# ATTron/astroz

Measured on AMD Instinct MI355X. Metric: propagations/sec, 13,478 sats x 1,440 times, at 1/2/4/8 MI355X, higher is better.
Workload: dtype f64

## Files before the change

astroz_amd/_native.py:

```python
import ctypes as C
import os

import numpy as np

_HERE = os.path.dirname(os.path.abspath(__file__))
LIB_PATH = os.environ.get("ASTROZ_AMD_LIB") or os.path.join(_HERE, "libastroz_hip.so")

WGS84, WGS72 = 0, 1
OUT_TEME, OUT_ECEF, OUT_GEODETIC, OUT_TOPOCENTRIC = 0, 1, 2, 3
SAT_MAJOR, TIME_MAJOR = 0, 1
OUTPUT_MODES = {"teme": OUT_TEME, "ecef": OUT_ECEF, "geodetic": OUT_GEODETIC, "topocentric": OUT_TOPOCENTRIC}
PASS_DTYPE = np.dtype([("t_rise_min", "<f8"), ("t_culm_min", "<f8"), ("t_set_min", "<f8"), ("max_elevation_rad", "<f8"),
                       ("rise_azimuth_rad", "<f8"), ("set_azimuth_rad", "<f8"), ("flags", "<u4"), ("grid_rise", "<u4"),
                       ("grid_culm", "<u4"), ("grid_set", "<u4")])
PASS_UP_AT_START, PASS_UP_AT_END, PASS_CUT_BY_ERROR = 1, 2, 4
ECLIPSE_DTYPE = np.dtype([("t_entry_min", "<f8"), ("t_exit_min", "<f8"), ("flags", "<u4"), ("grid_entry", "<u4"),
                          ("grid_exit", "<u4"), ("reserved", "<u4")])
ECLIPSE_IN_AT_START, ECLIPSE_IN_AT_END, ECLIPSE_CUT_BY_ERROR = 1, 2, 4
SHADOW_UMBRA, SHADOW_PENUMBRA = 0, 1
SHADOW_KINDS = {"umbra": SHADOW_UMBRA, "penumbra": SHADOW_PENUMBRA}
ACCESS_DTYPE = np.dtype([("t_start_min", "<f8"), ("t_end_min", "<f8"), ("min_range_km", "<f8"), ("flags", "<u4"),
                         ("grid_start", "<u4"), ("grid_end", "<u4"), ("grid_min_range", "<u4")])
ACCESS_OPEN_AT_START, ACCESS_OPEN_AT_END, ACCESS_CUT_BY_ERROR = 1, 2, 4
CONJUNCTION_DTYPE = np.dtype([("t_tca_min", "<f8"), ("miss_km", "<f8"), ("rel_speed_km_s", "<f8"), ("target", "<u4"),
                              ("sat", "<u4"), ("grid_index", "<u4"), ("reserved", "<u4")])

COVERAGE_DTYPE = np.dtype([("mean_in_view", "<f8"), ("max_gap_min", "<f8"), ("n_covered", "<u4"), ("min_in_view", "<u4"),
                           ("max_in_view", "<u4"), ("n_gaps", "<u4"), ("grid_gap_start", "<u4"), ("grid_gap_end", "<u4"),
                           ("flags", "<u4"), ("reserved", "<u4")])
COVERAGE_GAP_AT_START, COVERAGE_GAP_AT_END = 1, 2

AZ_ERR_HIP = -200
PATH_ROWS_FAST, PATH_TILES_FAST, PATH_ROWS_GENERIC, PATH_LANE_SAT, PATH_DEEP_ROWS, PATH_QUASI_UNIFORM, PATH_COLS_FAST, PATH_HOST_STEP = 1, 2, 4, 8, 16, 32, 64, 128

EXPORTS = [
    "astroz_version", "astroz_init", "astroz_deinit", "tle_parse", "tle_free",
    "tle_get_satellite_number", "tle_get_epoch", "tle_get_inclination", "tle_get_eccentricity",
    "tle_get_mean_motion", "sgp4_init", "sgp4_free", "sgp4_propagate", "sgp4_propagate_batch",
    "azh_device_count", "azh_last_error", "azh_parse_tle_lines", "azh_constellation_from_tle_text",
    "azh_constellation_from_tle_lines", "azh_constellation_from_elements", "azh_constellation_subset", "azh_constellation_free",
    "azh_num_satellites", "azh_num_sgp4", "azh_num_sdp4", "azh_get_epochs", "azh_get_status",
    "azh_get_field", "azh_propagate_host", "azh_propagate_device", "azh_propagate_device_cached", "azh_propagate_device_window",
    "azh_propagate_jd_host", "azh_synchronize", "azh_propagate_one_host", "azh_set_time_tile", "azh_set_timing", "azh_set_fast_path", "azh_set_tile_kernel", "azh_set_graphs", "azh_set_f32_arithmetic", "azh_set_f32_mode",
    "azh_last_kernel_ms", "azh_last_path", "azh_last_one_stats", "azh_last_window_tiers", "azh_set_host_copy_threads", "azh_set_host_points", "azh_get_host_points", "azh_selftest_coords", "azh_selftest_host_step", "azh_host_alloc", "azh_host_free", "azh_host_pool_stats", "azh_host_pool_trim", "azh_propagate_device_f32", "azh_propagate_device_cached_f32",
    "azh_screen_target_host", "azh_screen_target_device", "azh_coarse_screen_device", "azh_coarse_screen_host",
    "azh_screen_all_host", "azh_constellation_from_omm_json", "azh_propagate_one_device", "azh_selftest_math",
    "azh_parse_tle_text", "azh_parse_omm_json", "azh_set_parse_threads", "coords_julian_to_gmst",
    "azh_group_create_from_tle_text", "azh_group_create_from_omm_json", "azh_group_free", "azh_group_num_satellites",
    "azh_group_num_devices", "azh_group_padded_rows", "azh_group_get_epochs", "azh_group_propagate_host",
    "azh_group_propagate_allgather", "azh_group_screen_target_host", "azh_group_screen_target_device", "azh_group_shard_size",
    "azh_group_shard_rows", "azh_group_synchronize", "azh_screen_track_device", "coords_eci_to_ecef", "coords_ecef_to_geodetic",
    "orbital_hohmann", "orbital_velocity", "orbital_period", "orbital_escape_velocity",
    "azh_coords_topocentric", "azh_set_observer", "azh_find_passes_host", "azh_find_passes_device",
    "azh_find_passes_stations_host", "azh_find_passes_stations_device",
    "azh_coverage_host", "azh_coverage_device",
    "azh_sun_position_teme", "azh_selftest_sun", "azh_shadow_state", "azh_find_eclipses_host", "azh_find_eclipses_device",
    "azh_line_of_sight", "azh_find_access_host", "azh_find_access_device", "azh_find_access_track_device",
    "azh_closest_approach", "azh_find_conjunctions_host", "azh_find_conjunctions_device",
]


def _stations(stations, min_elevation_deg):
    st = np.ascontiguousarray(stations, dtype=np.float64).reshape(-1, 3)
    mk = np.ascontiguousarray(np.broadcast_to(np.asarray(min_elevation_deg, dtype=np.float64), (len(st),)))
    return st, mk


def _targets(targets):
    a = np.atleast_1d(np.asarray(targets))
    if a.ndim != 1 or a.size == 0 or a.dtype == np.bool_ or not np.issubdtype(a.dtype, np.integer) or (a < 0).any():
        raise ValueError("targets must be a satellite index or a non-empty sequence of them")
    return np.ascontiguousarray(a, dtype=np.uintp)


def _min_satellites(k):
    if isinstance(k, bool) or not isinstance(k, (int, np.integer)) or not 1 <= int(k) <= 0xFFFFFFFF:
        raise ValueError("min_satellites must be an integer >= 1")
# ... 143 lines not shown
    L.azh_set_timing.restype = i32
    L.azh_set_fast_path.argtypes = [vp, i32]
    L.azh_set_fast_path.restype = i32
    L.azh_set_tile_kernel.argtypes = [vp, i32]
    L.azh_set_tile_kernel.restype = i32
    L.azh_set_graphs.argtypes = [vp, i32]
    L.azh_set_graphs.restype = i32
    L.azh_set_f32_arithmetic.argtypes = [vp, i32]
    L.azh_set_f32_arithmetic.restype = i32
    L.azh_set_f32_mode.argtypes = [vp, i32]
    L.azh_set_f32_mode.restype = i32
    L.azh_last_kernel_ms.argtypes = [vp]
    L.azh_last_kernel_ms.restype = dbl
    L.azh_set_host_copy_threads.argtypes = [i32]
    L.azh_set_host_copy_threads.restype = None
    L.azh_set_host_points.argtypes = [sz]
    L.azh_set_host_points.restype = None
    L.azh_get_host_points.argtypes = []
    L.azh_get_host_points.restype = sz
    L.azh_host_alloc.argtypes = [C.c_size_t, C.POINTER(C.c_void_p)]
    L.azh_host_alloc.restype = i32
    L.azh_host_free.argtypes = [C.c_void_p]
    L.azh_host_free.restype = None
    L.azh_host_pool_stats.argtypes = [C.POINTER(C.c_size_t), C.POINTER(C.c_size_t)]
    L.azh_host_pool_stats.restype = None
    L.azh_host_pool_trim.argtypes = []
    L.azh_host_pool_trim.restype = None
    L.azh_last_path.argtypes = [vp]
    L.azh_last_path.restype = u32
    L.azh_last_one_stats.argtypes = [vp, vp, vp]
    L.azh_last_one_stats.restype = C.c_int32
    L.azh_last_window_tiers.argtypes = [vp, vp]
    L.azh_last_window_tiers.restype = C.c_int32
    L.azh_propagate_device_f32.argtypes = L.azh_propagate_device.argtypes
    L.azh_propagate_device_f32.restype = i32
    L.azh_propagate_device_cached_f32.argtypes = L.azh_propagate_device_cached.argtypes
    L.azh_propagate_device_cached_f32.restype = i32
    L.azh_screen_target_host.argtypes = [vp, vp, sz, vp, sz, dbl, dbl, vp, vp]
    L.azh_screen_target_host.restype = i32
    L.azh_screen_target_device.argtypes = [vp, vp, sz, vp, sz, dbl, dbl, vp, vp, vp]
    L.azh_screen_target_device.restype = i32
    L.azh_screen_track_device.argtypes = [vp, vp, sz, vp, vp, sz, dbl, vp, vp, vp]
    L.azh_screen_track_device.restype = i32
    L.azh_coarse_screen_device.argtypes = [vp, sz, sz, i32, sz, dbl, vp, vp, vp, sz, C.POINTER(sz), vp]
    L.azh_coarse_screen_device.restype = i32
    L.azh_coarse_screen_host.argtypes = [vp, sz, sz, i32, sz, dbl, vp, vp, vp, sz, C.POINTER(sz), i32]
    L.azh_coarse_screen_host.restype = i32
    L.azh_screen_all_host.argtypes = [vp, vp, sz, vp, dbl, vp, vp, sz, C.POINTER(sz)]
    L.azh_screen_all_host.restype = i32
    L.azh_coords_topocentric.argtypes = [vp, vp, dbl, vp, vp, vp]
    L.azh_coords_topocentric.restype = None
    L.azh_set_observer.argtypes = [vp, dbl, dbl, dbl]
    L.azh_set_observer.restype = i32
    L.azh_find_passes_host.argtypes = [vp, vp, sz, vp, dbl, dbl, vp, sz, vp]
    L.azh_find_passes_host.restype = i32
    L.azh_find_passes_device.argtypes = [vp, vp, sz, vp, dbl, dbl, vp, sz, vp, vp]
    L.azh_find_passes_device.restype = i32
    L.azh_find_passes_stations_host.argtypes = [vp, vp, sz, vp, dbl, vp, vp, sz, vp, sz, vp]
    L.azh_find_passes_stations_host.restype = i32
    L.azh_find_passes_stations_device.argtypes = [vp, vp, sz, vp, dbl, vp, vp, sz, vp, sz, vp, vp]
    L.azh_find_passes_stations_device.restype = i32
    L.azh_coverage_host.argtypes = [vp, vp, sz, vp, dbl, vp, vp, sz, u32, vp, vp]
    L.azh_coverage_host.restype = i32
    L.azh_coverage_device.argtypes = [vp, vp, sz, vp, dbl, vp, vp, sz, u32, vp, vp, vp]
    L.azh_coverage_device.restype = i32
    L.azh_sun_position_teme.argtypes = [dbl, vp]
# ... 381 lines not shown

    def set_fast_path(self, enabled):
        check(lib().azh_set_fast_path(self._h, 1 if enabled else 0), "azh_set_fast_path")

    def set_tile_kernel(self, enabled):
        check(lib().azh_set_tile_kernel(self._h, int(enabled) if not isinstance(enabled, bool) else (1 if enabled else 0)), "azh_set_tile_kernel")

    def set_graphs(self, enabled):
        check(lib().azh_set_graphs(self._h, 1 if enabled else 0), "azh_set_graphs")

    def set_timing(self, enabled):
        check(lib().azh_set_timing(self._h, 1 if enabled else 0), "azh_set_timing")

    def synchronize(self):
        check(lib().azh_synchronize(self._h), "azh_synchronize")

    def last_kernel_ms(self):
        return lib().azh_last_kernel_ms(self._h)

    def last_path(self):
        return int(lib().azh_last_path(self._h))

    def last_one_stats(self):
        a, b = C.c_uint32(0), C.c_uint32(0)
        check(lib().azh_last_one_stats(self._h, C.byref(a), C.byref(b)), "azh_last_one_stats")
        return int(a.value), int(b.value)


    def last_window_tiers(self):
        cnt = (C.c_uint32 * 4)()
        check(lib().azh_last_window_tiers(self._h, cnt), "azh_last_window_tiers")
        return dict(zip(("general", "eps", "ecc", "rejected"), (int(x) for x in cnt)))


class DeviceGroup:

    def __init__(self, text, devices, grav=WGS72, n_chunks=4):
        b = text.encode() if isinstance(text, str) else bytes(text)
        dv = (C.c_int32 * len(devices))(*devices)
        h = C.c_void_p()
        fn = lib().azh_group_create_from_omm_json if b.lstrip()[:1] in (b"{", b"[") else lib().azh_group_create_from_tle_text
        check(fn(b, len(b), grav, dv, len(devices), n_chunks, C.byref(h)), "azh_group_create")
        self._h = h
        self.n = lib().azh_group_num_satellites(h)
        self.n_devices = lib().azh_group_num_devices(h)
        self.padded_rows = lib().azh_group_padded_rows(h)
        self.epochs = np.empty(self.n)
        check(lib().azh_group_get_epochs(h, self.epochs.ctypes.data), "azh_group_get_epochs")

    def close(self):
        if getattr(self, "_h", None):
            lib().azh_group_free(self._h)
            self._h = None

    def __del__(self):
        try:
            self.close()
        except Exception:
            pass

    def _offsets(self, offsets_min):
        if offsets_min is None:
            return None
        off = _f64(offsets_min)
        if off.ndim != 1 or len(off) < self.n:
            raise ValueError("epoch_offsets must have at least num_satellites elements")
# ... 271 lines not shown
```

astroz_amd/csrc/astroz_hip.hip:

```cpp
#include "../../include/astroz_hip.h"

#include <hip/hip_runtime.h>
#include <dlfcn.h>
#include <rccl/rccl.h>

#include <algorithm>
#include <atomic>
#include <cmath>
#include <condition_variable>
#include <deque>
#include <map>
#include <cstdio>
#include <cstdlib>
#include <cstring>
#include <mutex>
#include <new>
#include <memory>
#include <string>
#include <thread>
#include <type_traits>
#include <vector>

#include "kernels.h"
#include "passes_kernel.h"
// ... 3059 lines not shown
    unsigned head[AZ_ONE_HEAD];
    HIP_TRY(hipMemcpy(head, c->d_one_items.p, sizeof(head), hipMemcpyDeviceToHost));
    unsigned cnt = 0;
    for (unsigned k = 0; k < AZ_ONE_LISTS; ++k) cnt += head[32u * k];
    *n_handed_over = cnt;
    return AZ_OK;
}

int32_t azh_last_window_tiers(azh_constellation *c, uint32_t counts[AZH_WINDOW_TIER_COUNTS])
{
    if (!c || !counts) return AZ_ERR_NULL_POINTER;
    for (unsigned k = 0; k < AZH_WINDOW_TIER_COUNTS; ++k) counts[k] = 0;
    if (c->last_plan < 0 || !c->plan[c->last_plan].valid) return AZ_OK;
    const azh_constellation::FastPlan &pl = c->plan[c->last_plan];
    if (set_device(c) != AZ_OK) return AZ_ERR_HIP;
    HIP_TRY(hipDeviceSynchronize());
    std::vector<unsigned char> f;
    try {
        f.resize((size_t)pl.n_list * pl.n_seg);
    } catch (const std::bad_alloc &) {
        return AZ_ERR_HIP;
    }
    if (f.empty()) return AZ_OK;
    HIP_TRY(hipMemcpy(f.data(), pl.flag.p, f.size(), hipMemcpyDeviceToHost));
    for (unsigned char v : f) {
        if (!(v & AZ_PLAN_SET)) continue;
        if (!(v & AZ_PLAN_OK)) ++counts[AZH_WINDOW_TIER_REJECTED];
        else if (v & AZ_PLAN_ECC) ++counts[AZH_WINDOW_TIER_ECC];
        else ++counts[((v >> AZ_PLAN_TIER_SHIFT) & AZ_PLAN_TIER_MASK) ? AZH_WINDOW_TIER_EPS : AZH_WINDOW_TIER_GENERAL];
    }
    return AZ_OK;
}

double azh_last_kernel_ms(azh_constellation *c)
{
    if (!c || !c->timed) return -1.0;
    float ms = -1.0f;
    if (hipEventElapsedTime(&ms, c->ev_t0, c->ev_t1) != hipSuccess) {
        (void)hipGetLastError();
        return -1.0;
    }
    return (double)ms;
}

int32_t azh_propagate_one_host(azh_constellation *c, size_t sat, const double *tsince, size_t n, double *pos,
                               double *vel, uint8_t *err)
{
    return guarded([&]() -> int32_t {
        if (!c || !tsince || !pos) return AZ_ERR_NULL_POINTER;
        if (sat >= c->n) return AZ_ERR_VALUE;
        if (n == 0) return AZ_OK;
        return run_one_satellite(c, sat, tsince, n, 0, nullptr, pos, vel, err);
    });
}

int32_t azh_propagate_one_device(azh_constellation *c, size_t sat, const double *d_tsince, size_t n, double *d_pos,
                                 double *d_vel, uint8_t *d_err, void *stream)
{
    return guarded([&]() -> int32_t {
        if (!c || !d_tsince || !d_pos) return AZ_ERR_NULL_POINTER;
        if (sat >= c->n || n > 0xffffffffu) return AZ_ERR_VALUE;
        if (n == 0) return AZ_OK;
        if (set_device(c) != AZ_OK) return AZ_ERR_HIP;
        hipStream_t st = stream ? (hipStream_t)stream : c->s_main;
        if (c->timing) HIP_TRY(hipEventRecord(c->ev_t0, st));
        if (int32_t lrc = launch_one(c, sat, d_tsince, n, d_pos, d_vel, d_err, 0, st); lrc != AZ_OK) return lrc;
// ... 670 lines not shown
```

astroz_amd/csrc/fast_step.h:

```cpp
#pragma once
#include <type_traits>

#include "propagate_device.h"

#define AZ_FASTK_COLD(X)                                                                                     \
    X(cc1) X(d2) X(d3) X(d4) X(nl2) X(nl3) X(nl4) X(nl5) X(eta) X(omgcof) X(xmcof) X(xd) X(bc4) X(bc5) X(ecb) X(sab)
#define AZ_FASTK_HOT(X)                                                                                      \
    X(aycof) X(xlcof) X(xnodcf) X(sinio) X(cosio) X(k_mrt) X(k_c2u) X(k_su) X(k_node) X(k_inc) X(x1mth2) X(k_rv) \
    X(sdA) X(cdA) X(sdW) X(cdW) X(tc) X(sdU) X(cdU) X(tmid) X(nodedot) X(sOc) X(cOc)
enum FastCold {
#define X(n) FC_##n,
    AZ_FASTK_COLD(X)
#undef X
    FC_NUM
};
#define AZ_FASTK_DELTA(X) X(mdot) X(argpdot) X(udot)
enum FastColdX {
    FCX_first_ = FC_NUM - 1,
#define X(n) FCX_##n,
    AZ_FASTK_DELTA(X)
#undef X
    FCX_NUM
};
#define AZ_DELTA_MAX 4.0e-6
// ... 270 lines not shown
            "v_fma_f64 %0, %0, %5, %2\n\t"
            "v_fma_f64 %1, %1, %5, -%3"
            : "+v"(s), "+v"(c), "=&v"(m), "=&v"(m2)
            : "s"(sd), "s"(cd));
        return;
    }
#endif
    const double ns = fma(s, cd, c * sd);
    c = fma(c, cd, -(s * sd));
    s = ns;
}

template <class RC>
AZ_DEVICE void az_pq_ecc_scaled(double d, const RC &k, double &p, double &q)
{
    const double d2 = d * d;
    q = d2 * fma(d2, k(RC_p24), -0.5);
    p = d * fma(d2, fma(d2, k(RC_p120), k(RC_n6)), 1.0);
}
template <class RC>
AZ_DEVICE void az_fpq_milli(double d, const RC &k, double &p, double &q)
{
    const double d2 = d * d;
    q = d2 * fma(d2, k(RC_p24), -0.5);
    p = fma(d2 * k(RC_n6), d, d);
}

#define AZ_FAST_EL2 1.6e-5
#define AZ_FAST_TEMP2 6.0e-4

enum { AZ_TIER_GENERAL = 0, AZ_TIER_EPS = 1, AZ_TIER_NUM = 2 };
#define AZ_TIER_EPS_MAX 0.0009765625
#define AZ_FAST_EM_MIN 1.0e-6

template <bool ECC>
AZ_DEVICE int az_fast_window_tier(const FastK &k, const AzGrav &g, double t_a, double t_b, double dmax = 0.0)
{
    const double T = fmax(fabs(t_a), fabs(t_b)) + dmax;
    const double ae = fabs(k.eta_);
    const double th = fma(fabs(k.xmcof_), ae * fma(2.0 * ae, ae, 6.0), fabs(k.omgcof_) * T);
    const double da = T * fma(T, fma(T, fma(T, fabs(k.d4_), fabs(k.d3_)), fabs(k.d2_)), fabs(k.cc1_));
    const double dem = fma(fabs(k.bc4_), T, fabs(k.bc5_));
    const double em = fabs(k.ecb_) + dem;
    bool ok = (th <= AZ_ROT_16TH) & (da <= 0.25) & (em <= 0.9);
    ok &= k.ecb_ - dem >= AZ_FAST_EM_MIN;
    const double sam = k.sab_ * (1.0 - da);
    const double inv_am = 1.0 / (sam * sam);
    const double temp = inv_am / fma(-em, em, 1.0);
    const double el = fma(temp, fabs(k.aycof_), em);
    const double el2 = el * el;
    if (!ECC) ok &= el2 <= AZ_FAST_EL2;
    ok &= el2 <= 0.81;
    const double dc = fmax(fabs(t_a - k.tc_), fabs(t_b - k.tc_)) + dmax;
    const double eps = fma(temp * fabs(k.xlcof_), em, fma(fabs(k.nl2_) * dc, dc, T * T * T * fma(T, fma(T, fabs(k.nl5_), fabs(k.nl4_)), fabs(k.nl3_)))) +
                       fabs(k.udot_) * dmax;
    ok &= eps <= AZ_ROT_MED;
    const double inv_pl = inv_am / (1.0 - el2);
    const double temp2 = g.half_j2 * inv_pl * inv_pl;
    ok &= temp2 <= AZ_FAST_TEMP2;
    const double a_nd = fma(fabs(k.k_node_), temp2, fma(fabs(k.nodedot_), 0.5 * fabs(t_b - t_a) + dmax, fabs(k.xnodcf_) * T * T));
    ok &= a_nd <= AZ_ROT_MED;
    if (!ok) return -1;
    return (!ECC && eps <= AZ_TIER_EPS_MAX) ? AZ_TIER_EPS : AZ_TIER_GENERAL;
}
template <bool ECC>
AZ_DEVICE bool az_fast_window_ok(const FastK &k, const AzGrav &g, double t_a, double t_b, double dmax = 0.0)
{
    return az_fast_window_tier<ECC>(k, g, t_a, t_b, dmax) >= 0;
}

#ifndef AZ_FAST_PROBE
#define AZ_FAST_PROBE(name, value)
#endif

template <bool VEL, bool ECC = false, int DELTA = 0, int TIER = AZ_TIER_GENERAL, class K = FastK, class RC = RotCoefLit>
AZ_DEVICE bool az_sgp4_fast_step(const K &k, const AzGrav &g, const RC &rk, double t, FastCarry &st, double r[3],
                                  double v[3], double dl = 0.0)
{
    az_pair_advance<K::SCALAR>(st.sA, st.cA, k.sdA(), k.cdA());
    az_pair_advance<K::SCALAR>(st.sW, st.cW, k.sdW(), k.cdW());
    az_pair_advance<K::SCALAR>(st.sU, st.cU, k.sdU(), k.cdU());
    double sA = st.sA, cA = st.cA, sW = st.sW, cW = st.cW;
    if constexpr ((DELTA == 1 && ECC) || DELTA == 2) {
        const double a = k.mdot() * dl, b = k.argpdot() * dl;
        if constexpr (DELTA == 2 && ECC) {
            double pa, qa;
            az_pq_16th(a, rk, pa, qa);
            az_rot_apply2(sA, cA, pa, qa);
        } else if constexpr (DELTA == 2) {
            az_rotate_tiny2(sA, cA, a, rk);
        } else {
            sA = fma(st.cA, a, st.sA); cA = fma(-st.sA, a, st.cA);
        }
        if constexpr (DELTA == 2 && ECC) az_rotate_tiny2(sW, cW, b, rk);
        else { sW = fma(st.cW, b, st.sW); cW = fma(-st.sW, b, st.cW); }
    }
    const double t2 = t * t;

    const double dm = fma(k.eta(), cA, 1.0);
    const double th = fma(k.xmcof(), dm * dm * dm, fma(k.omgcof(), t, -k.xd()));
    const double tempa = fma(-t, fma(t, fma(t, fma(t, k.d4(), k.d3()), k.d2()), k.cc1()), 1.0);
    const double dtc = t - k.tc();
    double nl = fma(k.nl2() * dtc, dtc, t2 * (t * fma(t, fma(t, k.nl5(), k.nl4()), k.nl3())));
    if constexpr (DELTA != 0) nl = fma(k.udot(), dl, nl);
    bool bad = false;
    double p, q;
    if (ECC) az_pq_16th(th, rk, p, q);
    else az_pq_ecc_scaled(th, rk, p, q);
    const double smm = fma(cA, p, fma(sA, q, sA));
    const double sw = fma(-cW, p, fma(sW, q, sW));
    const double cw = fma(sW, p, fma(cW, q, cW));
    const double em = fma(-k.bc5(), smm, fma(-k.bc4(), t, k.ecb()));
    AZ_FAST_PROBE(th, th)
    AZ_FAST_PROBE(em, em)

    const double sqrt_am = k.sab() * fabs(tempa);
    const double am = sqrt_am * sqrt_am;
    const double omem2 = fma(-em, em, 1.0);
    const double R = az_rcp(sqrt_am * omem2);
    const double ra = R * omem2;
    const double temp = ra * R;

    const double axnl = em * cw;
    const double aynl = fma(em, sw, temp * k.aycof());
    double s = st.sU, c = st.cU;
    {
        const double eps = fma(temp * k.xlcof(), axnl, nl);
        AZ_FAST_PROBE(eps, eps)
        if constexpr (!ECC && TIER >= AZ_TIER_EPS) az_rotate_tiny2(s, c, eps, rk);
        else {
            az_pq_16th(eps, rk, p, q);
            az_rot_apply2(s, c, p, q);
        }
    }

    const double el2 = fma(axnl, axnl, aynl * aynl);
    double ecose, esine, ome, inv_ome, betal, inv_omel2, inv_1pb;
    if (!ECC) {
        const double rden = az_rcp1(fma(-s, aynl, fma(-c, axnl, 1.0)));
        const double d0 = fma(axnl, s, -(aynl * c)) * rden;
        az_fpq_milli(d0, rk, p, q);
        az_rot_apply2(s, c, p, q);
        const double d1 = fma(axnl, s, fma(-aynl, c, -d0)) * rden;
        {
            const double s1 = fma(c, d1, s);
            c = fma(-s, d1, c);
            s = s1;
        }
        ecose = fma(axnl, c, aynl * s);
        esine = fma(axnl, s, -(aynl * c));
        ome = 1.0 - ecose;
        const double x = fma(-ome, rden, 1.0);
        inv_ome = fma(rden, fma(x, x, x), rden);
        betal = fma(el2, fma(el2, -0.125, -0.5), 1.0);
        inv_omel2 = el2 + 1.0;
        inv_1pb = fma(el2, rk(RC_p8), 0.5);
    } else {
        double eps = 0.0, rden = 1.0, d = 0.0;
#pragma unroll
        for (int it = 0; it < 5; ++it) {
            rden = az_rcp1(fma(-s, aynl, fma(-c, axnl, 1.0)));
            d = fma(axnl, s, fma(-aynl, c, -eps)) * rden;
            eps += d;
            if (it == 0) {
                bad |= !(fabs(d) <= 0.5);
                az_pq_large(d, rk, p, q);
                az_rot_apply2(s, c, p, q);
            } else if (it == 1) {
                bad |= !(fabs(d) <= AZ_ROT_MED);
                az_pq_med(d, rk, p, q);
                az_rot_apply2(s, c, p, q);
            } else {
                bad |= !(fabs(d) <= AZ_ROT_SMALL);
                az_fpq_small(d, rk, p, q);
                az_rot_apply2(s, c, p, q);
            }
        }
        const double d2 = d * d;
        bad |= !(el2 * d2 * d2 < 4.0e-26);
        ecose = fma(axnl, c, aynl * s);
        esine = fma(axnl, s, -(aynl * c));
        ome = 1.0 - ecose;
        inv_ome = fma(rden, fma(-ome, rden, 1.0), rden);
        const double omel2 = 1.0 - el2;
        const double rb = az_rsqrt(omel2);
        betal = omel2 * rb;
        inv_omel2 = rb * rb;
        inv_1pb = az_rcp(1.0 + betal);
    }
// ... 43 lines not shown
```

astroz_amd/csrc/kernels.h:

```cpp
#pragma once
#include <hip/hip_runtime.h>

#include <type_traits>

#include "init_device.h"
#include "propagate_device.h"
#include "fast_step.h"
#include "fast_step_f32.h"

#ifndef AZ_BLOCK
#define AZ_BLOCK 256
#endif
#ifndef AZ_PROP_FAST
#define AZ_PROP_FAST 1
#endif
#ifndef AZ_MIN_WAVES
#define AZ_MIN_WAVES 1
#endif
#ifndef AZ_ROWS_WAVES
#define AZ_ROWS_WAVES 3
#endif
#ifndef AZ_DEEP_WAVES
#define AZ_DEEP_WAVES 2
#endif
// ... 34 lines not shown
    double uniform_step;
    int grid_exact_uniform;
    const float *delta;
    double delta_max;
    const double *delta64;
    int delta_wide;
    double grid_t0;
    const double *inc;
    const double *fast_rec;
    unsigned row_lo, row_hi;
    unsigned slot_lo, slot_hi;
    unsigned win_circ_lo, win_circ_hi, win_ecc_lo, win_ecc_hi;
    int arith32;
    unsigned n_circ;
    unsigned redo_slot0;
    unsigned *redo_count;
    unsigned *redo_next;
    unsigned *redo_items;
    const unsigned *rowmap;
    const double *tmp_pos, *tmp_vel;
    unsigned n_rows;
    const double *plan_win;
    const unsigned char *plan_flag;
    unsigned plan_stride;
    const unsigned *redo_static;
    AzGrav g;
};
enum { AZ_ROW_NEAR = 0, AZ_ROW_COPY = 1, AZ_ROW_ZERO = 2 };
enum { AZ_PLAN_sOc, AZ_PLAN_cOc, AZ_PLAN_sdU, AZ_PLAN_cdU, AZ_PLAN_s1U, AZ_PLAN_c1U, AZ_PLAN_NUM };
#define AZ_PLAN_OK 1u
#define AZ_PLAN_TC 2u
#define AZ_PLAN_TIER_SHIFT 2
#define AZ_PLAN_TIER_MASK 1u
#define AZ_PLAN_ECC 16u
#define AZ_PLAN_SET 32u

template <class T>
__device__ __forceinline__ void az_put3(T *o, const double r[3])
{
    o[0] = (T)r[0];
    o[1] = (T)r[1];
    o[2] = (T)r[2];
}
typedef double az_d2s __attribute__((ext_vector_type(2), aligned(8)));
typedef float az_f3s __attribute__((ext_vector_type(3), aligned(4)));
#ifndef AZ_ROWS_NT
#define AZ_ROWS_NT 1
#endif
__device__ __forceinline__ void az_put3_stream(double *o, const double r[3])
{
#if AZ_ROWS_NT
    const az_d2s a = {r[0], r[1]};
    __builtin_nontemporal_store(a, reinterpret_cast<az_d2s *>(o));
    __builtin_nontemporal_store(r[2], o + 2);
#else
    az_put3(o, r);
#endif
}
__device__ __forceinline__ void az_put3_stream(float *o, const double r[3])
{
#if AZ_ROWS_NT
    const az_f3s a = {(float)r[0], (float)r[1], (float)r[2]};
    __builtin_nontemporal_store(a, reinterpret_cast<az_f3s *>(o));
#else
    az_put3(o, r);
#endif
// ... 421 lines not shown
    const unsigned *flags;
    size_t n_pad;
    const unsigned *list;
    unsigned n_list, n_circ, n_times, tile_c, tile_e, by_flags;
    unsigned f32_mixed;
    const double *times, *offsets, *inc;
    double step, dt_mult, delta_max, grid_t0;
    double *win;
    unsigned char *flag;
    unsigned *redo_static, *redo_c0, *redo_c1, *redo_items;
    AzGrav g;
};
__global__ void __launch_bounds__(256) k_plan_windows(PlanArgs a)
{
    const unsigned slot = blockIdx.x * 256 + threadIdx.x;
    const unsigned seg = blockIdx.y;
    if (slot >= a.n_list) return;
    const unsigned s = a.list[slot];
    const unsigned fl = a.flags[s];
    const bool ecc = a.by_flags ? AZ_FLAG_ECLASS(fl) != 0 : slot >= a.n_circ;
    const unsigned tile = ecc ? a.tile_e : a.tile_c;
    const unsigned t_lo = seg * tile;
    if (t_lo >= a.n_times) return;
    const unsigned t_hi = min(t_lo + tile, a.n_times);
    const double t_first = a.grid_t0 + (a.offsets ? a.offsets[s] : 0.0);
    const double w_a = fma((double)t_lo, a.step, t_first), w_b = fma((double)(t_hi - 1), a.step, t_first);
    FastK k0, k1;
    az_load_fast(a.el, a.n_pad, s, fl, a.inc, 0, k0);
    const double dt_mult = ecc ? 64.0 : a.dt_mult;
    if (dt_mult == 128.0) az_double_increments(k0);
    az_fast_window(a.el, a.n_pad, s, w_a, w_b, dt_mult * a.step, k0);
    az_load_fast(a.el, a.n_pad, s, fl, a.inc, 1, k1);
    az_fast_window(a.el, a.n_pad, s, w_a, w_b, a.step, k1);
    const int tier = ecc ? az_fast_window_tier<true>(k0, a.g, w_a, w_b, a.delta_max) : az_fast_window_tier<false>(k0, a.g, w_a, w_b, a.delta_max);
    bool ok = tier >= 0;
    if (!ecc && AZ_FLAG_ECLASS(fl) != 0) ok = false;
    if (!ecc && a.f32_mixed && !az_fast32p_window_ok(k0, w_a, w_b)) ok = false;
    const size_t at = (size_t)seg * a.n_list + slot;
    double *w = a.win + at * AZ_PLAN_NUM;
    w[AZ_PLAN_sOc] = k0.sOc_; w[AZ_PLAN_cOc] = k0.cOc_; w[AZ_PLAN_sdU] = k0.sdU_; w[AZ_PLAN_cdU] = k0.cdU_;
    w[AZ_PLAN_s1U] = k1.sdU_; w[AZ_PLAN_c1U] = k1.cdU_;
    a.flag[at] = (unsigned char)((ok ? AZ_PLAN_OK | ((unsigned)tier << AZ_PLAN_TIER_SHIFT) : 0u) | (k0.tc_ != 0.0 ? AZ_PLAN_TC : 0u) |
                                 (ecc ? AZ_PLAN_ECC : 0u) | AZ_PLAN_SET);
    if (!ok) {
        const unsigned k = atomicAdd(a.redo_static, 1u);
        a.redo_items[3 * (size_t)k + 0] = slot;
        a.redo_items[3 * (size_t)k + 1] = t_lo;
        a.redo_items[3 * (size_t)k + 2] = t_hi;
    }
}
__global__ void k_plan_arm(unsigned *redo_static, unsigned *c0, unsigned *c1)
{
    if (threadIdx.x == 0 && blockIdx.x == 0) *c0 = *c1 = *redo_static;
}
template <class K>
__device__ __forceinline__ bool az_plan_window(const PropArgs &p, unsigned seg, unsigned slot, double w_a, double w_b, K &k0, unsigned *tier = nullptr)
{
    const size_t at = (size_t)seg * p.plan_stride + slot;
    const double *w = p.plan_win + at * AZ_PLAN_NUM;
    const unsigned f = p.plan_flag[at];
    k0.tmid_ = 0.5 * (w_a + w_b);
    k0.tc_ = (f & AZ_PLAN_TC) ? k0.tmid_ : 0.0;
    k0.sOc_ = w[AZ_PLAN_sOc]; k0.cOc_ = w[AZ_PLAN_cOc]; k0.sdU_ = w[AZ_PLAN_sdU]; k0.cdU_ = w[AZ_PLAN_cdU];
    if (tier) *tier = (f >> AZ_PLAN_TIER_SHIFT) & AZ_PLAN_TIER_MASK;
    return (f & AZ_PLAN_OK) != 0;
}

AZ_DEVICE double az_uniform(double x)
{
#ifdef AZ_HOST_EMUL
    return x;
#else
    return __hiloint2double(__builtin_amdgcn_readfirstlane(__double2hiint(x)),
                            __builtin_amdgcn_readfirstlane(__double2loint(x)));
#endif
}
AZ_DEVICE float az_uniform32(float x)
{
#ifdef AZ_HOST_EMUL
    return x;
#else
    return __int_as_float(__builtin_amdgcn_readfirstlane(__float_as_int(x)));
#endif
}
__device__ __forceinline__ const double *az_opaque_lds(const double *p)
{
    typedef __attribute__((address_space(3))) const double lds_cdouble;
    lds_cdouble *q = (lds_cdouble *)p;
    asm volatile("" : "+v"(q));
    return (const double *)q;
}
struct ColdBroadcast;
struct ColdBroadcast {
    double *p;
    const double *m = nullptr;
    __device__ __forceinline__ double operator()(int k) const { return p[k]; }
    __device__ __forceinline__ void set(int k, double v) const { p[k] = v; }
// ... 297 lines not shown
                const double dx = q[0] - r[0], dy = q[1] - r[1], dz = q[2] - r[2];
                const double d2 = fma(dx, dx, fma(dy, dy, dz * dz));
                if (live && d2 < best_d2) {
                    best_d2 = d2;
                    best_t = i;
                }
                continue;
            }
            if (FRAME) {
                if (((base - t_lo) & (AZ_FRAME_SEG - 1u)) == 0u && base != t_lo) {
                    az_wave_lds_fence();
#pragma unroll
                    for (unsigned j = lane; j < AZ_FRAME_SEG; j += 64) {
                        const unsigned jn = min(base + j, p.n_times - 1);
                        gst_lds[2 * j] = p.sin_g[jn];
                        gst_lds[2 * j + 1] = p.cos_g[jn];
                    }
                    az_wave_lds_fence();
                }
                const unsigned jj = (i - t_lo) & (AZ_FRAME_SEG - 1u);
                const double sg = gst_lds[2 * jj], cg = gst_lds[2 * jj + 1];
                az_to_ecef(r, sg, cg);
                if (VEL) az_to_ecef(v, sg, cg);
                if (FRAME == 2) az_ecef_to_geodetic(r);
                if (FRAME == 3) az_topocentric<VEL>(r, v, obs);
            }
#if defined(AZ_ABLATE) && AZ_ABLATE == 1
            if (!(live && (r[0] + r[1] + r[2] + (VEL ? v[0] + v[1] + v[2] : 0.0)) == 1.2345e300)) continue;
#endif
            az_rows_store<VEL>(staged, base + 64 <= t_hi, live, lane, rows_stage, prow, vrow, base, r, v, sink);
        }
        };
        if constexpr (AZ_ROWS_TIERS && !ECC && FRAME == 0) run(std::integral_constant<int, AZ_TIER_EPS>(), tier == AZ_TIER_EPS ? t_hi : t_lo);
        run(std::integral_constant<int, AZ_TIER_GENERAL>(), t_hi);
    }
    if (SINK == AZ_SINK_SCREEN) {
        az_wave_argmin(best_d2, best_t);
        if (lane == 0) {
            p.part_d2[(size_t)blockIdx.y * p.plan_stride + row + p.redo_slot0] = best_d2;
            p.part_t[(size_t)blockIdx.y * p.plan_stride + row + p.redo_slot0] = best_t;
        }
    }
    if (ECC && base < t_hi && lane == 0) {
        const unsigned k = atomicAdd(p.redo_count, 1u);
        p.redo_items[3 * (size_t)k + 0] = row + p.redo_slot0;
        p.redo_items[3 * (size_t)k + 1] = base;
        p.redo_items[3 * (size_t)k + 2] = t_hi;
    }
}

#define AZ_TILE_SATS 16
#define AZ_TILE_SEG_MAX 1024
#define AZ_TILE_PITCH 49
template <bool VEL, int FRAME = 0, int DELTA = 0>
__global__ void __launch_bounds__(1024, 1) k_tiles_fast(PropArgs p)
{
    constexpr unsigned NA = VEL ? 2u : 1u;
    constexpr bool ECEF = FRAME != 0;
    [[maybe_unused]] const AzObserver obs = FRAME == 3 ? *p.obs : AzObserver{};
    __shared__ __attribute__((aligned(16))) double cold_all[AZ_TILE_SATS * AZ_FAST_TABLE];
    __shared__ __attribute__((aligned(16))) double tile[2 * NA * 64 * AZ_TILE_PITCH];
    __shared__ double gst[ECEF ? 2 * AZ_TILE_SEG_MAX : 2];
    const unsigned lane = threadIdx.x & 63u, w = __builtin_amdgcn_readfirstlane(threadIdx.x >> 6);
    double *cold_lds = cold_all + w * AZ_FAST_TABLE;
    const unsigned tile_id = az_xcd_row();
    const unsigned s_first = tile_id * AZ_TILE_SATS;
// ... 893 lines not shown
```

bindings/zig/astroz_hip.zig:

```

pub const HipError = error{
    BadTleLength,
    BadChecksum,
    DeepSpaceNotSupported,
    InvalidEccentricity,
    SatelliteDecayed,
    ValueError,
    OutOfMemory,
    NullPointer,
    NotInitialized,
    DeviceFailure,
    Unknown,
};

pub fn check(rc: i32) HipError!void {
    return switch (rc) {
        0 => {},
        -1 => HipError.BadTleLength,
        -2 => HipError.BadChecksum,
        -10 => HipError.DeepSpaceNotSupported,
        -11 => HipError.InvalidEccentricity,
        -12 => HipError.SatelliteDecayed,
        -20 => HipError.ValueError,
        -100 => HipError.OutOfMemory,
// ... 58 lines not shown
    d_track: [*]const f64, exclude_index: usize, threshold_km: f64, d_min_dist_km: [*]f64, d_min_t_index: [*]u32, stream: ?*anyopaque) i32;
pub extern "c" fn azh_coarse_screen_device(d_pos: [*]const f64, n_sats: usize, n_times: usize, layout: i32, stride_sats: usize,
    threshold_km: f64, valid_mask: ?[*]const u8, out_pairs: [*]u32, out_t_index: [*]u32, max_results: usize, n_found: *usize,
    stream: ?*anyopaque) i32;
pub extern "c" fn azh_coarse_screen_host(pos: [*]const f64, n_sats: usize, n_times: usize, layout: i32, stride_sats: usize,
    threshold_km: f64, valid_mask: ?[*]const u8, out_pairs: [*]u32, out_t_index: [*]u32, max_results: usize, n_found: *usize,
    device: i32) i32;
pub extern "c" fn azh_screen_all_host(h: ?*Handle, times_min: [*]const f64, n_times: usize, epoch_offsets_min: ?[*]const f64,
    threshold_km: f64, out_pairs: [*]u32, out_t_index: [*]u32, max_results: usize, n_found: *usize) i32;

pub extern "c" fn azh_parse_tle_text(text: [*]const u8, len: usize, out16: [*]f64, max_records: usize, n_found: *usize) i32;
pub extern "c" fn azh_parse_omm_json(text: [*]const u8, len: usize, out16: [*]f64, max_records: usize, n_found: *usize) i32;
pub extern "c" fn azh_set_parse_threads(n: i32) void;
pub extern "c" fn azh_constellation_from_omm_json(text: [*]const u8, len: usize, grav: i32, device: i32, out: *?*Handle) i32;
pub extern "c" fn azh_constellation_subset(h: ?*const Handle, indices: [*]const u32, n: usize, device: i32, out: *?*Handle) i32;

pub extern "c" fn azh_propagate_device_window(h: ?*Handle, row_lo: usize, row_hi: usize, d_pos: [*]f64, d_vel: ?[*]f64, layout: i32,
    out_stride_sats: usize, d_err: ?[*]u8, stream: ?*anyopaque) i32;
pub extern "c" fn azh_set_f32_mode(h: ?*Handle, mode: i32) i32;
pub extern "c" fn azh_set_f32_arithmetic(h: ?*Handle, enabled: i32) i32;
pub extern "c" fn azh_set_fast_path(h: ?*Handle, enabled: i32) i32;
pub extern "c" fn azh_set_tile_kernel(h: ?*Handle, enabled: i32) i32;
pub extern "c" fn azh_set_graphs(h: ?*Handle, enabled: i32) i32;
pub extern "c" fn azh_set_host_points(n: usize) void;
pub extern "c" fn azh_get_host_points() usize;
pub extern "c" fn azh_set_host_copy_threads(n: i32) void;
pub extern "c" fn azh_host_alloc(bytes: usize, out: *?*anyopaque) i32;
pub extern "c" fn azh_host_free(p: ?*anyopaque) void;
pub extern "c" fn azh_host_pool_stats(live_bytes: ?*usize, free_bytes: ?*usize) void;
pub extern "c" fn azh_host_pool_trim() void;
pub extern "c" fn azh_last_path(h: ?*const Handle) u32;
pub extern "c" fn azh_last_one_stats(h: ?*Handle, n_segments: ?*u32, n_handed_over: ?*u32) i32;
pub extern "c" fn azh_last_window_tiers(h: ?*Handle, counts: *[4]u32) i32;
pub extern "c" fn azh_propagate_one_device(h: ?*Handle, sat_index: usize, d_tsince_min: [*]const f64, n: usize, d_pos: [*]f64,
    d_vel: ?[*]f64, d_err: ?[*]u8, stream: ?*anyopaque) i32;
pub extern "c" fn azh_selftest_math(x: [*]const f64, n: usize, out6n: [*]f64, device: i32) i32;
pub extern "c" fn azh_selftest_host_step(el: [*]const f64, n_pad: usize, sat: usize, flags: u32, grav: i32, tsince_min: [*]const f64, n: usize,
    out6n: [*]f64, err: ?[*]u8) i32;
pub extern "c" fn azh_selftest_coords(op: i32, in: *const [4]f64, out: *[5]f64) i32;

pub extern "c" fn coords_julian_to_gmst(jd: f64) f64;
pub extern "c" fn coords_eci_to_ecef(eci: *const [3]f64, gmst: f64, ecef: *[3]f64) void;
pub extern "c" fn coords_ecef_to_geodetic(ecef: *const [3]f64, lla: *[3]f64) void;
pub extern "c" fn azh_coords_topocentric(r_teme: *const [3]f64, v_teme: ?*const [3]f64, gmst: f64, observer_lla: *const [3]f64,
    aer: *[3]f64, aer_rate: ?*[3]f64) void;

pub const OUT_TOPOCENTRIC: i32 = 3;
pub const Pass = extern struct {
    t_rise_min: f64,
    t_culm_min: f64,
    t_set_min: f64,
    max_elevation_rad: f64,
    rise_azimuth_rad: f64,
    set_azimuth_rad: f64,
    flags: u32,
    grid_rise: u32,
    grid_culm: u32,
    grid_set: u32,
};
pub const PASS_UP_AT_START: u32 = 1;
pub const PASS_UP_AT_END: u32 = 2;
pub const PASS_CUT_BY_ERROR: u32 = 4;
pub extern "c" fn azh_set_observer(h: ?*Handle, lat_deg: f64, lon_deg: f64, alt_km: f64) i32;
pub extern "c" fn azh_find_passes_host(h: ?*Handle, times_min: [*]const f64, n_times: usize, epoch_offsets_min: ?[*]const f64,
    reference_jd: f64, min_elevation_deg: f64, out: [*]Pass, max_passes: usize, n_passes: [*]u32) i32;
pub extern "c" fn azh_find_passes_device(h: ?*Handle, times_min: [*]const f64, n_times: usize, epoch_offsets_min: ?[*]const f64,
// ... 114 lines not shown
```

include/astroz_hip.h:

```cpp
#ifndef ASTROZ_HIP_H
#define ASTROZ_HIP_H

#include <stddef.h>
#include <stdint.h>

#ifdef __cplusplus
extern "C" {
#endif

enum {
    AZ_OK = 0,
    AZ_ERR_BAD_TLE_LENGTH = -1,
    AZ_ERR_BAD_CHECKSUM = -2,
    AZ_ERR_DEEP_SPACE_NOT_SUPPORTED = -10,
    AZ_ERR_INVALID_ECCENTRICITY = -11,
    AZ_ERR_SATELLITE_DECAYED = -12,
    AZ_ERR_VALUE = -20,
    AZ_ERR_ALLOC_FAILED = -100,
    AZ_ERR_NULL_POINTER = -101,
    AZ_ERR_NOT_INITIALIZED = -102,
    AZ_ERR_HIP = -200,
    AZ_ERR_UNKNOWN = -999
};

// ... 259 lines not shown
int32_t azh_selftest_coords(int32_t op, const double in[4], double out[5]);
int32_t azh_selftest_host_step(const double *el, size_t n_pad, size_t sat, uint32_t flags, int32_t grav, const double *tsince_min,
                               size_t n, double *out6n, uint8_t *err);

int32_t azh_set_time_tile(azh_constellation *c, uint32_t sgp4_tile, uint32_t sdp4_tile);
int32_t azh_set_fast_path(azh_constellation *c, int32_t enabled);
int32_t azh_set_tile_kernel(azh_constellation *c, int32_t enabled);
int32_t azh_set_graphs(azh_constellation *c, int32_t enabled);
void azh_set_host_copy_threads(int32_t n);
void azh_set_host_points(size_t n);
size_t azh_get_host_points(void);
int32_t azh_host_alloc(size_t bytes, void **out);
void azh_host_free(void *p);
void azh_host_pool_stats(size_t *live_bytes, size_t *free_bytes);
void azh_host_pool_trim(void);
int32_t azh_set_timing(azh_constellation *c, int32_t enabled);
double azh_last_kernel_ms(azh_constellation *c);
#define AZH_PATH_ROWS_FAST 1u
#define AZH_PATH_TILES_FAST 2u
#define AZH_PATH_ROWS_GENERIC 4u
#define AZH_PATH_LANE_SAT 8u
#define AZH_PATH_DEEP_ROWS 16u
#define AZH_PATH_COLS_FAST 64u
#define AZH_PATH_QUASI_UNIFORM 32u
#define AZH_PATH_HOST_STEP 128u
uint32_t azh_last_path(const azh_constellation *c);
int32_t azh_last_one_stats(azh_constellation *c, uint32_t *n_segments, uint32_t *n_handed_over);
#define AZH_WINDOW_TIER_GENERAL 0
#define AZH_WINDOW_TIER_EPS 1
#define AZH_WINDOW_TIER_ECC 2
#define AZH_WINDOW_TIER_REJECTED 3
#define AZH_WINDOW_TIER_COUNTS 4
int32_t azh_last_window_tiers(azh_constellation *c, uint32_t counts[AZH_WINDOW_TIER_COUNTS]);

#ifdef __cplusplus
}
#endif
#endif
```

Baseline: 95.71 billion.

## Add eccentricity tiers with specialized Kepler solvers for ECC fast path

```diff
diff --git a/astroz_amd/_native.py b/astroz_amd/_native.py
--- a/astroz_amd/_native.py
+++ b/astroz_amd/_native.py
@@ -42,7 +42,7 @@
     "azh_num_satellites", "azh_num_sgp4", "azh_num_sdp4", "azh_get_epochs", "azh_get_status",
     "azh_get_field", "azh_propagate_host", "azh_propagate_device", "azh_propagate_device_cached", "azh_propagate_device_window",
     "azh_propagate_jd_host", "azh_synchronize", "azh_propagate_one_host", "azh_set_time_tile", "azh_set_timing", "azh_set_fast_path", "azh_set_tile_kernel", "azh_set_graphs", "azh_set_f32_arithmetic", "azh_set_f32_mode",
-    "azh_last_kernel_ms", "azh_last_path", "azh_last_one_stats", "azh_last_window_tiers", "azh_set_host_copy_threads", "azh_set_host_points", "azh_get_host_points", "azh_selftest_coords", "azh_selftest_host_step", "azh_host_alloc", "azh_host_free", "azh_host_pool_stats", "azh_host_pool_trim", "azh_propagate_device_f32", "azh_propagate_device_cached_f32",
+    "azh_last_kernel_ms", "azh_last_path", "azh_last_one_stats", "azh_last_window_tiers", "azh_last_window_ecc_tiers", "azh_set_host_copy_threads", "azh_set_host_points", "azh_get_host_points", "azh_selftest_coords", "azh_selftest_host_step", "azh_host_alloc", "azh_host_free", "azh_host_pool_stats", "azh_host_pool_trim", "azh_propagate_device_f32", "azh_propagate_device_cached_f32",
     "azh_screen_target_host", "azh_screen_target_device", "azh_coarse_screen_device", "azh_coarse_screen_host",
     "azh_screen_all_host", "azh_constellation_from_omm_json", "azh_propagate_one_device", "azh_selftest_math",
     "azh_parse_tle_text", "azh_parse_omm_json", "azh_set_parse_threads", "coords_julian_to_gmst",
@@ -252,6 +252,8 @@
     L.azh_last_one_stats.restype = C.c_int32
     L.azh_last_window_tiers.argtypes = [vp, vp]
     L.azh_last_window_tiers.restype = C.c_int32
+    L.azh_last_window_ecc_tiers.argtypes = [vp, vp]
+    L.azh_last_window_ecc_tiers.restype = C.c_int32
     L.azh_propagate_device_f32.argtypes = L.azh_propagate_device.argtypes
     L.azh_propagate_device_f32.restype = i32
     L.azh_propagate_device_cached_f32.argtypes = L.azh_propagate_device_cached.argtypes
@@ -699,6 +701,11 @@
         check(lib().azh_last_window_tiers(self._h, cnt), "azh_last_window_tiers")
         return dict(zip(("general", "eps", "ecc", "rejected"), (int(x) for x in cnt)))
 
+    def last_window_ecc_tiers(self):
+        cnt = (C.c_uint32 * 3)()
+        check(lib().azh_last_window_ecc_tiers(self._h, cnt), "azh_last_window_ecc_tiers")
+        return dict(zip(("e1", "e2", "general"), (int(x) for x in cnt)))
+
 
 class DeviceGroup:
 
diff --git a/astroz_amd/csrc/astroz_hip.hip b/astroz_amd/csrc/astroz_hip.hip
--- a/astroz_amd/csrc/astroz_hip.hip
+++ b/astroz_amd/csrc/astroz_hip.hip
@@ -3115,6 +3115,30 @@
     return AZ_OK;
 }
 
+int32_t azh_last_window_ecc_tiers(azh_constellation *c, uint32_t counts[AZH_WINDOW_ECC_COUNTS])
+{
+    if (!c || !counts) return AZ_ERR_NULL_POINTER;
+    for (unsigned k = 0; k < AZH_WINDOW_ECC_COUNTS; ++k) counts[k] = 0;
+    if (c->last_plan < 0 || !c->plan[c->last_plan].valid) return AZ_OK;
+    const azh_constellation::FastPlan &pl = c->plan[c->last_plan];
+    if (set_device(c) != AZ_OK) return AZ_ERR_HIP;
+    HIP_TRY(hipDeviceSynchronize());
+    std::vector<unsigned char> f;
+    try {
+        f.resize((size_t)pl.n_list * pl.n_seg);
+    } catch (const std::bad_alloc &) {
+        return AZ_ERR_HIP;
+    }
+    if (f.empty()) return AZ_OK;
+    HIP_TRY(hipMemcpy(f.data(), pl.flag.p, f.size(), hipMemcpyDeviceToHost));
+    for (unsigned char v : f) {
+        if ((v & (AZ_PLAN_SET | AZ_PLAN_OK | AZ_PLAN_ECC)) != (AZ_PLAN_SET | AZ_PLAN_OK | AZ_PLAN_ECC)) continue;
+        const unsigned t = (v >> AZ_PLAN_TIER_SHIFT) & AZ_PLAN_ETIER_MASK;
+        ++counts[t == AZ_ETIER_E1 ? AZH_WINDOW_ECC_E1 : (t == AZ_ETIER_E2 ? AZH_WINDOW_ECC_E2 : AZH_WINDOW_ECC_GENERAL)];
+    }
+    return AZ_OK;
+}
+
 double azh_last_kernel_ms(azh_constellation *c)
 {
     if (!c || !c->timed) return -1.0;
diff --git a/astroz_amd/csrc/fast_step.h b/astroz_amd/csrc/fast_step.h
--- a/astroz_amd/csrc/fast_step.h
+++ b/astroz_amd/csrc/fast_step.h
@@ -326,6 +326,10 @@
 enum { AZ_TIER_GENERAL = 0, AZ_TIER_EPS = 1, AZ_TIER_NUM = 2 };
 #define AZ_TIER_EPS_MAX 0.0009765625
 #define AZ_FAST_EM_MIN 1.0e-6
+
+enum { AZ_ETIER_E1 = 1, AZ_ETIER_E2 = 2, AZ_ETIER_NUM = 3 };
+#define AZ_ETIER_E1_MAX 0.01
+#define AZ_ETIER_E2_MAX 0.1
 
 template <bool ECC>
 AZ_DEVICE int az_fast_window_tier(const FastK &k, const AzGrav &g, double t_a, double t_b, double dmax = 0.0)
@@ -355,7 +359,8 @@
     const double a_nd = fma(fabs(k.k_node_), temp2, fma(fabs(k.nodedot_), 0.5 * fabs(t_b - t_a) + dmax, fabs(k.xnodcf_) * T * T));
     ok &= a_nd <= AZ_ROT_MED;
     if (!ok) return -1;
-    return (!ECC && eps <= AZ_TIER_EPS_MAX) ? AZ_TIER_EPS : AZ_TIER_GENERAL;
+    if (ECC) return el <= AZ_ETIER_E1_MAX ? (int)AZ_ETIER_E1 : (el <= AZ_ETIER_E2_MAX ? (int)AZ_ETIER_E2 : (int)AZ_TIER_GENERAL);
+    return eps <= AZ_TIER_EPS_MAX ? AZ_TIER_EPS : AZ_TIER_GENERAL;
 }
 template <bool ECC>
 AZ_DEVICE bool az_fast_window_ok(const FastK &k, const AzGrav &g, double t_a, double t_b, double dmax = 0.0)
@@ -365,6 +370,9 @@
 
 #ifndef AZ_FAST_PROBE
 #define AZ_FAST_PROBE(name, value)
+#endif
+#ifndef AZ_FAST_PROBE_KEPLER
+#define AZ_FAST_PROBE_KEPLER(name, value)
 #endif
 
 template <bool VEL, bool ECC = false, int DELTA = 0, int TIER = AZ_TIER_GENERAL, class K = FastK, class RC = RotCoefLit>
@@ -390,6 +398,7 @@
         else { sW = fma(st.cW, b, st.sW); cW = fma(-st.sW, b, st.cW); }
     }
     const double t2 = t * t;
+    constexpr bool E1 = ECC && TIER == AZ_ETIER_E1, E2 = ECC && TIER == AZ_ETIER_E2;
 
     const double dm = fma(k.eta(), cA, 1.0);
     const double th = fma(k.xmcof(), dm * dm * dm, fma(k.omgcof(), t, -k.xd()));
@@ -399,7 +408,8 @@
     if constexpr (DELTA != 0) nl = fma(k.udot(), dl, nl);
     bool bad = false;
     double p, q;
-    if (ECC) az_pq_16th(th, rk, p, q);
+    if (E1) az_fpq_small(th, rk, p, q);
+    else if (ECC) az_pq_16th(th, rk, p, q);
     else az_pq_ecc_scaled(th, rk, p, q);
     const double smm = fma(cA, p, fma(sA, q, sA));
     const double sw = fma(-cW, p, fma(sW, q, sW));
@@ -430,25 +440,65 @@
 
     const double el2 = fma(axnl, axnl, aynl * aynl);
     double ecose, esine, ome, inv_ome, betal, inv_omel2, inv_1pb;
-    if (!ECC) {
+    AZ_FAST_PROBE_KEPLER(el2, el2)
+    if (!ECC || E1) {
         const double rden = az_rcp1(fma(-s, aynl, fma(-c, axnl, 1.0)));
         const double d0 = fma(axnl, s, -(aynl * c)) * rden;
-        az_fpq_milli(d0, rk, p, q);
+        AZ_FAST_PROBE_KEPLER(d0, d0)
+        if (E1) az_pq_ecc_scaled(d0, rk, p, q);
+        else az_fpq_milli(d0, rk, p, q);
         az_rot_apply2(s, c, p, q);
         const double d1 = fma(axnl, s, fma(-aynl, c, -d0)) * rden;
+        AZ_FAST_PROBE_KEPLER(d1, d1)
         {
             const double s1 = fma(c, d1, s);
             c = fma(-s, d1, c);
+            s = s1;
+        }
+        if (E1) {
+            const double d2 = fma(axnl, s, fma(-aynl, c, -(d0 + d1))) * rden;
+            AZ_FAST_PROBE_KEPLER(d2, d2)
+            const double s1 = fma(c, d2, s);
+            c = fma(-s, d2, c);
             s = s1;
         }
         ecose = fma(axnl, c, aynl * s);
         esine = fma(axnl, s, -(aynl * c));
         ome = 1.0 - ecose;
         const double x = fma(-ome, rden, 1.0);
-        inv_ome = fma(rden, fma(x, x, x), rden);
+        inv_ome = fma(rden, E1 ? fma(x, fma(x, x, x), x) : fma(x, x, x), rden);
         betal = fma(el2, fma(el2, -0.125, -0.5), 1.0);
         inv_omel2 = el2 + 1.0;
+        if (E1) inv_omel2 = fma(el2, inv_omel2, 1.0);
         inv_1pb = fma(el2, rk(RC_p8), 0.5);
+    } else if (E2) {
+        double rden = az_rcp1(fma(-s, aynl, fma(-c, axnl, 1.0)));
+        const double d0 = fma(axnl, s, -(aynl * c)) * rden;
+        AZ_FAST_PROBE_KEPLER(d0, d0)
+        az_pq_med(d0, rk, p, q);
+        az_rot_apply2(s, c, p, q);
+        rden = az_rcp1(fma(-s, aynl, fma(-c, axnl, 1.0)));
+        const double d1 = fma(axnl, s, fma(-aynl, c, -d0)) * rden;
+        AZ_FAST_PROBE_KEPLER(d1, d1)
+        az_fpq_milli(d1, rk, p, q);
+        az_rot_apply2(s, c, p, q);
+        rden = az_rcp1(fma(-s, aynl, fma(-c, axnl, 1.0)));
+        const double d2 = fma(axnl, s, fma(-aynl, c, -(d0 + d1))) * rden;
+        AZ_FAST_PROBE_KEPLER(d2, d2)
+        {
+            const double s1 = fma(c, d2, s);
+            c = fma(-s, d2, c);
+            s = s1;
+        }
+        ecose = fma(axnl, c, aynl * s);
+        esine = fma(axnl, s, -(aynl * c));
+        ome = 1.0 - ecose;
+        inv_ome = fma(rden, fma(-ome, rden, 1.0), rden);
+        const double omel2 = 1.0 - el2;
+        const double rb = az_rsqrt(omel2);
+        betal = omel2 * rb;
+        inv_omel2 = rb * rb;
+        inv_1pb = az_rcp(1.0 + betal);
     } else {
         double eps = 0.0, rden = 1.0, d = 0.0;
 #pragma unroll
diff --git a/astroz_amd/csrc/kernels.h b/astroz_amd/csrc/kernels.h
--- a/astroz_amd/csrc/kernels.h
+++ b/astroz_amd/csrc/kernels.h
@@ -90,6 +90,10 @@
 #define AZ_PLAN_TC 2u
 #define AZ_PLAN_TIER_SHIFT 2
 #define AZ_PLAN_TIER_MASK 1u
+#define AZ_PLAN_ETIER_MASK 3u
+#ifndef AZ_ROWS_ETIERS
+#define AZ_ROWS_ETIERS 1
+#endif
 #define AZ_PLAN_ECC 16u
 #define AZ_PLAN_SET 32u
 
@@ -577,7 +581,8 @@
     az_fast_window(a.el, a.n_pad, s, w_a, w_b, dt_mult * a.step, k0);
     az_load_fast(a.el, a.n_pad, s, fl, a.inc, 1, k1);
     az_fast_window(a.el, a.n_pad, s, w_a, w_b, a.step, k1);
-    const int tier = ecc ? az_fast_window_tier<true>(k0, a.g, w_a, w_b, a.delta_max) : az_fast_window_tier<false>(k0, a.g, w_a, w_b, a.delta_max);
+    int tier = ecc ? az_fast_window_tier<true>(k0, a.g, w_a, w_b, a.delta_max) : az_fast_window_tier<false>(k0, a.g, w_a, w_b, a.delta_max);
+    if (ecc && (AZ_ROWS_ETIERS == 0 || (AZ_ROWS_ETIERS == 2 && tier == AZ_ETIER_E2))) tier = min(tier, (int)AZ_TIER_GENERAL);
     bool ok = tier >= 0;
     if (!ecc && AZ_FLAG_ECLASS(fl) != 0) ok = false;
     if (!ecc && a.f32_mixed && !az_fast32p_window_ok(k0, w_a, w_b)) ok = false;
@@ -607,7 +612,7 @@
     k0.tmid_ = 0.5 * (w_a + w_b);
     k0.tc_ = (f & AZ_PLAN_TC) ? k0.tmid_ : 0.0;
     k0.sOc_ = w[AZ_PLAN_sOc]; k0.cOc_ = w[AZ_PLAN_cOc]; k0.sdU_ = w[AZ_PLAN_sdU]; k0.cdU_ = w[AZ_PLAN_cdU];
-    if (tier) *tier = (f >> AZ_PLAN_TIER_SHIFT) & AZ_PLAN_TIER_MASK;
+    if (tier) *tier = (f >> AZ_PLAN_TIER_SHIFT) & ((f & AZ_PLAN_ECC) ? AZ_PLAN_ETIER_MASK : AZ_PLAN_TIER_MASK);
     return (f & AZ_PLAN_OK) != 0;
 }
 
@@ -971,6 +976,10 @@
         }
         };
         if constexpr (AZ_ROWS_TIERS && !ECC && FRAME == 0) run(std::integral_constant<int, AZ_TIER_EPS>(), tier == AZ_TIER_EPS ? t_hi : t_lo);
+        if constexpr (AZ_ROWS_ETIERS && ECC && FRAME == 0 && DELTA != 2) {
+            run(std::integral_constant<int, AZ_ETIER_E1>(), tier == AZ_ETIER_E1 ? t_hi : t_lo);
+            if constexpr (AZ_ROWS_ETIERS == 1) run(std::integral_constant<int, AZ_ETIER_E2>(), tier == AZ_ETIER_E2 ? t_hi : t_lo);
+        }
         run(std::integral_constant<int, AZ_TIER_GENERAL>(), t_hi);
     }
     if (SINK == AZ_SINK_SCREEN) {
diff --git a/bindings/zig/astroz_hip.zig b/bindings/zig/astroz_hip.zig
--- a/bindings/zig/astroz_hip.zig
+++ b/bindings/zig/astroz_hip.zig
@@ -114,6 +114,7 @@
 pub extern "c" fn azh_last_path(h: ?*const Handle) u32;
 pub extern "c" fn azh_last_one_stats(h: ?*Handle, n_segments: ?*u32, n_handed_over: ?*u32) i32;
 pub extern "c" fn azh_last_window_tiers(h: ?*Handle, counts: *[4]u32) i32;
+pub extern "c" fn azh_last_window_ecc_tiers(h: ?*Handle, counts: *[3]u32) i32;
 pub extern "c" fn azh_propagate_one_device(h: ?*Handle, sat_index: usize, d_tsince_min: [*]const f64, n: usize, d_pos: [*]f64,
     d_vel: ?[*]f64, d_err: ?[*]u8, stream: ?*anyopaque) i32;
 pub extern "c" fn azh_selftest_math(x: [*]const f64, n: usize, out6n: [*]f64, device: i32) i32;
diff --git a/include/astroz_hip.h b/include/astroz_hip.h
--- a/include/astroz_hip.h
+++ b/include/astroz_hip.h
@@ -315,6 +315,11 @@
 #define AZH_WINDOW_TIER_REJECTED 3
 #define AZH_WINDOW_TIER_COUNTS 4
 int32_t azh_last_window_tiers(azh_constellation *c, uint32_t counts[AZH_WINDOW_TIER_COUNTS]);
+#define AZH_WINDOW_ECC_E1 0
+#define AZH_WINDOW_ECC_E2 1
+#define AZH_WINDOW_ECC_GENERAL 2
+#define AZH_WINDOW_ECC_COUNTS 3
+int32_t azh_last_window_ecc_tiers(azh_constellation *c, uint32_t counts[AZH_WINDOW_ECC_COUNTS]);
 
 #ifdef __cplusplus
 }
```

After: 96.98 billion (median of 6 runs). +1.3%, better.
